# Samirez/Visual_odometry

Hardware: AMD Instinct MI355X
Metric: frame-pairs/sec (1280x720, 2000 ORB feats) (higher is better)
Workload: dtype u8+f32+f64; 1 GPU; seeded synthetic 1280x720 drone flight (256 distinct rendered views, closed loop), 2000 ORB features/frame, 8 levels = BASELINE config 2; chunk of 257 consecutive frames -> 256 pairs (k, k+1) per GPU per step, each frame detected once; detector=orb, distinct_rendered_frames=256, pair_stride=1, contexts_per_gpu=3, keypoint_order=cv2, poly_solver=fast, matcher=crosscheck, matcher_kernel=mfma_fp4, ransac=5-point, conf 0.99, 1 px, seed 2^64-1, <=1000 iters, parallelism=single GPU, pairs_ok_last_step=256

## Files before the change

### visual_odometry_amd/csrc/match_kernels.hip

```cpp
#include "vo_internal.h"
#include <float.h>
#include <limits.h>

#define NN_TILE 256

struct Desc { uint4 a, b; };

__device__ __forceinline__ int hamming(const Desc& x, const uint4& ya, const uint4& yb)
{
    return __popc(x.a.x ^ ya.x) + __popc(x.a.y ^ ya.y) + __popc(x.a.z ^ ya.z) + __popc(x.a.w ^ ya.w) +
           __popc(x.b.x ^ yb.x) + __popc(x.b.y ^ yb.y) + __popc(x.b.z ^ yb.z) + __popc(x.b.w ^ yb.w);
}

#define NN_Q 2
#define NN_ROWS_PER_BLOCK (256 * NN_Q)

template <bool KNN2>
__device__ __forceinline__ void nn_body(const uint8_t* A, int na, const uint8_t* B, int nb,
                                        int* idx, int* dist, int* idx2, int* dist2)
{
    __shared__ uint4 s_b[NN_TILE * 2];
    const int tid = threadIdx.x;
    Desc me[NN_Q];
    int row[NN_Q];
// ... 165 lines not shown
            if (j0 + 16 > nb && j0 + li >= nb) cin = c_bad;
            v4i b[4], acc[MM_RB];
#pragma unroll
            for (int s = 0; s < 4; s++) b[s] = *(const v4i*)(sb + g * 4096 + (4 * s + lg) * 256 + li * 16);
#pragma unroll
            for (int rb = 0; rb < MM_RB; rb++) acc[rb] = __builtin_amdgcn_mfma_i32_16x16x64_i8(a[rb][0], b[0], cin, 0, 0, 0);
#pragma unroll
            for (int s = 1; s < 4; s++)
#pragma unroll
                for (int rb = 0; rb < MM_RB; rb++) acc[rb] = __builtin_amdgcn_mfma_i32_16x16x64_i8(a[rb][s], b[s], acc[rb], 0, 0, 0);
#pragma unroll
            for (int rb = 0; rb < MM_RB; rb++)
#pragma unroll
                for (int r = 0; r < 4; r++) {
                    const int key = acc[rb][r];
                    if (KNN2) best2[rb][r] = max(best2[rb][r], min(best[rb][r], key));
                    best[rb][r] = max(best[rb][r], key);
                }
        }
    }
#undef MM_GLDS

    const size_t o = ((size_t)p * 2 + dir) * kp_cap, o2 = (size_t)p * kp_cap;
#pragma unroll
    for (int rb = 0; rb < MM_RB; rb++)
#pragma unroll
        for (int r = 0; r < 4; r++) {
            int k0 = best[rb][r], k1 = best2[rb][r];
#pragma unroll
            for (int d = 1; d < 16; d <<= 1) {
                const int u0 = __shfl_xor(k0, d, 64), u1 = __shfl_xor(k1, d, 64);
                if (KNN2) k1 = max(max(k1, u1), min(k0, u0));
                k0 = max(k0, u0);
            }
            const int row = wrow0 + rb * 16 + lg * 4 + r;
            if (li == 0 && row < na) {
                pb.nn_idx[o + row] = k0 >= 0 ? MM_S - 1 - k0 % MM_S : -1;
                pb.nn_dist[o + row] = k0 >= 0 ? (512 - k0 / MM_S) >> 1 : INT_MAX;
                if (KNN2) {
                    pb.nn_idx2[o2 + row] = k1 >= 0 ? MM_S - 1 - k1 % MM_S : -1;
                    pb.nn_dist2[o2 + row] = k1 >= 0 ? (512 - k1 / MM_S) >> 1 : INT_MAX;
                }
            }
        }
}

typedef int v8i __attribute__((ext_vector_type(8)));
typedef float v4f __attribute__((ext_vector_type(4)));
#define MF_S 8192
#ifndef MF_STAGE_ROWS
#define MF_STAGE_ROWS 128
#endif
#define MF_LD (MF_STAGE_ROWS * 128 / 16 / MM_THREADS)
template <bool KNN2>
__global__ __launch_bounds__(MM_THREADS) void k_nn_fp4(const uint8_t* desc_x, const int* kp_count, int kp_cap, int cap_x,
                                                PairBuf pb, int dir_first, int row_blocks)
{
    __shared__ __attribute__((aligned(16))) uint8_t s_b[2][MF_STAGE_ROWS * 128];
    const int bid = xcd_tile(blockIdx.x, gridDim.x);
    const int p = bid / row_blocks, dir = dir_first + blockIdx.z;
    const int fa = pb.slots[2 * p + dir], fb = pb.slots[2 * p + (dir ^ 1)];
    const int na = min(kp_count[fa], kp_cap), nb = min(kp_count[fb], kp_cap);
    const int row0 = (bid % row_blocks) * MM_BLOCK_ROWS;
    if (row0 >= na) return;
    const int tid = threadIdx.x, lane = tid & 63, wave = __builtin_amdgcn_readfirstlane(tid >> 6);
    const int li = lane & 15, lg = lane >> 4;
    const uint8_t* A = desc_x + (size_t)fa * cap_x * 256;
    const uint8_t* B = desc_x + (size_t)fb * cap_x * 256;
    const int wrow0 = row0 + wave * MM_WAVE_ROWS;

    v8i a[MM_RB][2];
#pragma unroll
    for (int rb = 0; rb < MM_RB; rb++)
#pragma unroll
        for (int s = 0; s < 2; s++) {
            const v4i v = wrow0 < na ? *(const v4i*)(A + ((size_t)((wrow0 >> 4) + rb) * 8 + 4 * s + lg) * 256 + li * 16) : (v4i){0, 0, 0, 0};
            a[rb][s] = __builtin_shufflevector(v, v, 0, 1, 2, 3, -1, -1, -1, -1);
        }
    const float c_bad = -1.0e9f;
    const float c_lane = (float)(MF_S * 256 + (MF_S - 1) - li);
    v4i best[MM_RB], best2[MM_RB];
#pragma unroll
    for (int rb = 0; rb < MM_RB; rb++) { best[rb] = (v4i){INT_MIN, INT_MIN, INT_MIN, INT_MIN}; best2[rb] = best[rb]; }

    const int nstages = (nb + MF_STAGE_ROWS - 1) / MF_STAGE_ROWS;
    const bool active = wrow0 < na;
    v4f cin = {c_lane, c_lane, c_lane, c_lane};
#define MF_GLDS(stage, buf)                                                                                        \
    _Pragma("unroll") for (int q = 0; q < MF_LD; q++)                                                              \
        __builtin_amdgcn_global_load_lds((const __attribute__((address_space(1))) void*)(B + (size_t)(stage) * (MF_STAGE_ROWS * 128) + (size_t)(q * MM_THREADS + tid) * 16), \
                                         (__attribute__((address_space(3))) void*)(s_b[buf] + (q * MM_THREADS + wave * 64) * 16), 16, 0, 0)
    if (nstages > 0) { MF_GLDS(0, 0); }
    for (int sg = 0; sg < nstages; sg++) {
        asm volatile("s_waitcnt vmcnt(0)" ::: "memory");
        __syncthreads();
        if (sg + 1 < nstages) { MF_GLDS(sg + 1, (sg + 1) & 1); }
        const uint8_t* sb = s_b[sg & 1];
        const int first = sg * (MF_STAGE_ROWS / 16);
        const int ngf = active ? min(MF_STAGE_ROWS / 16, max((nb >> 4) - first, 0)) : 0;
        const bool tail = active && (nb & 15) && first + ngf == (nb >> 4) && ngf < MF_STAGE_ROWS / 16;
        auto group = [&](int g, const v4f& c, v4f (&acc)[MM_RB]) {
            v8i b[2];
#pragma unroll
            for (int s = 0; s < 2; s++) {
                const v4i v = *(const v4i*)(sb + g * 2048 + (4 * s + lg) * 256 + li * 16);
                b[s] = __builtin_shufflevector(v, v, 0, 1, 2, 3, -1, -1, -1, -1);
            }
#pragma unroll
            for (int rb = 0; rb < MM_RB; rb++) acc[rb] = __builtin_amdgcn_mfma_scale_f32_16x16x128_f8f6f4(a[rb][0], b[0], c, 4, 4, 0, 140, 0, 127);
#pragma unroll
            for (int rb = 0; rb < MM_RB; rb++) acc[rb] = __builtin_amdgcn_mfma_scale_f32_16x16x128_f8f6f4(a[rb][1], b[1], acc[rb], 4, 4, 0, 140, 0, 127);
        };
        const v4f sixteen = {16.f, 16.f, 16.f, 16.f};
        int g = 0;
        for (; g + 1 < ngf; g += 2) {
            v4f acc0[MM_RB], acc1[MM_RB];
            const v4f c1 = cin - sixteen;
            group(g, cin, acc0); group(g + 1, c1, acc1);
            cin = c1 - sixteen;
#pragma unroll
            for (int rb = 0; rb < MM_RB; rb++)
#pragma unroll
                for (int r = 0; r < 4; r++) {
                    const int k0 = __float_as_int(acc0[rb][r]), k1 = __float_as_int(acc1[rb][r]);
                    if (KNN2) {
                        best2[rb][r] = max(best2[rb][r], min(best[rb][r], k0));
                        best[rb][r] = max(best[rb][r], k0);
                        best2[rb][r] = max(best2[rb][r], min(best[rb][r], k1));
                        best[rb][r] = max(best[rb][r], k1);
                    } else best[rb][r] = max(max(best[rb][r], k0), k1);
                }
        }
        for (; g < ngf + (tail ? 1 : 0); g++) {
            v4f acc[MM_RB];
            v4f c = cin;
            if (g == ngf) { const float cm = (first + g) * 16 + li >= nb ? c_bad : cin[0]; c = (v4f){cm, cm, cm, cm}; }
            group(g, c, acc);
            cin = cin - sixteen;
#pragma unroll
            for (int rb = 0; rb < MM_RB; rb++)
#pragma unroll
                for (int r = 0; r < 4; r++) {
                    const int key = __float_as_int(acc[rb][r]);
                    if (KNN2) best2[rb][r] = max(best2[rb][r], min(best[rb][r], key));
                    best[rb][r] = max(best[rb][r], key);
                }
        }
    }
#undef MF_GLDS

    const size_t o = ((size_t)p * 2 + dir) * kp_cap, o2 = (size_t)p * kp_cap;
#pragma unroll
    for (int rb = 0; rb < MM_RB; rb++)
#pragma unroll
        for (int r = 0; r < 4; r++) {
            int k0 = best[rb][r], k1 = best2[rb][r];
#pragma unroll
            for (int d = 1; d < 16; d <<= 1) {
                const int u0 = __shfl_xor(k0, d, 64), u1 = __shfl_xor(k1, d, 64);
                if (KNN2) k1 = max(max(k1, u1), min(k0, u0));
                k0 = max(k0, u0);
            }
            const int row = wrow0 + rb * 16 + lg * 4 + r;
            if (li == 0 && row < na) {
                const int i0 = k0 >= 0 ? (int)__int_as_float(k0) : -1, i1 = k1 >= 0 ? (int)__int_as_float(k1) : -1;
                pb.nn_idx[o + row] = i0 >= 0 ? MF_S - 1 - (i0 & (MF_S - 1)) : -1;
                pb.nn_dist[o + row] = i0 >= 0 ? (512 - (i0 >> 13)) >> 1 : INT_MAX;
                if (KNN2) {
                    pb.nn_idx2[o2 + row] = i1 >= 0 ? MF_S - 1 - (i1 & (MF_S - 1)) : -1;
                    pb.nn_dist2[o2 + row] = i1 >= 0 ? (512 - (i1 >> 13)) >> 1 : INT_MAX;
                }
            }
        }
}

void launch_match_nn(hipStream_t s, const uint8_t* desc_x, const int* kp_count, int kp_cap, int cap_x, PairBuf pb, int P,
                     int dirs_mask, int knn2, int fp4)
{
    if (P <= 0) return;
    dim3 block(MM_THREADS);
    const int gx = (kp_cap + MM_BLOCK_ROWS - 1) / MM_BLOCK_ROWS;
    if (fp4) {
        if (knn2) hipLaunchKernelGGL(k_nn_fp4<true>, dim3(gx * P, 1, 1), block, 0, s, desc_x, kp_count, kp_cap, cap_x, pb, 0, gx);
        else if (dirs_mask == 3) hipLaunchKernelGGL(k_nn_fp4<false>, dim3(gx * P, 1, 2), block, 0, s, desc_x, kp_count, kp_cap, cap_x, pb, 0, gx);
        else hipLaunchKernelGGL(k_nn_fp4<false>, dim3(gx * P, 1, 1), block, 0, s, desc_x, kp_count, kp_cap, cap_x, pb, dirs_mask == 2 ? 1 : 0, gx);
        return;
    }
    if (knn2) {
        hipLaunchKernelGGL(k_nn_mfma<true>, dim3(gx * P, 1, 1), block, 0, s, desc_x, kp_count, kp_cap, cap_x, pb, 0, gx);
        return;
    }
    if (dirs_mask == 3) hipLaunchKernelGGL(k_nn_mfma<false>, dim3(gx * P, 1, 2), block, 0, s, desc_x, kp_count, kp_cap, cap_x, pb, 0, gx);
    else if (dirs_mask == 1) hipLaunchKernelGGL(k_nn_mfma<false>, dim3(gx * P, 1, 1), block, 0, s, desc_x, kp_count, kp_cap, cap_x, pb, 0, gx);
    else if (dirs_mask == 2) hipLaunchKernelGGL(k_nn_mfma<false>, dim3(gx * P, 1, 1), block, 0, s, desc_x, kp_count, kp_cap, cap_x, pb, 1, gx);
}

#define L8_STAGE_ROWS 128
#define L8_LD (L8_STAGE_ROWS * 128 / 16 / MM_THREADS)
template <bool KNN2, bool PACKED>
__device__ __forceinline__ void nn_l2i8_body(uint8_t (*s_b)[L8_STAGE_ROWS * 128], const uint8_t* desc_x, const int* norms, int kp_cap, int cap_x,
                                             const PairBuf& pb, int p, int dir, int fa, int fb, int na, int nb, int row0)
{
    constexpr bool packed = PACKED;
    const int tid = threadIdx.x, lane = tid & 63, wave = __builtin_amdgcn_readfirstlane(tid >> 6);
    const int li = lane & 15, lg = lane >> 4;
    const uint8_t* A = desc_x + (size_t)fa * cap_x * 128;
    const uint8_t* B = desc_x + (size_t)fb * cap_x * 128;
    const int* nB = norms + (size_t)fb * cap_x;
    const int wrow0 = row0 + wave * MM_WAVE_ROWS;

    v4i a[MM_RB][2];
#pragma unroll
    for (int rb = 0; rb < MM_RB; rb++)
#pragma unroll
        for (int s = 0; s < 2; s++)
            a[rb][s] = wrow0 < na ? *(const v4i*)(A + ((size_t)((wrow0 >> 4) + rb) * 8 + 4 * s + lg) * 256 + li * 16) : (v4i){0, 0, 0, 0};
    v4i bv[MM_RB], bg[MM_RB], bv2[MM_RB], bg2[MM_RB];
#pragma unroll
    for (int rb = 0; rb < MM_RB; rb++) { bv[rb] = (v4i){INT_MIN, INT_MIN, INT_MIN, INT_MIN}; bg[rb] = (v4i){-1, -1, -1, -1}; bv2[rb] = bv[rb]; bg2[rb] = bg[rb]; }

    const int nstages = (nb + L8_STAGE_ROWS - 1) / L8_STAGE_ROWS;
    const bool active = wrow0 < na;

#define L8_GLDS(stage, buf)                                                                                        \
    _Pragma("unroll") for (int q = 0; q < L8_LD; q++)                                                              \
        __builtin_amdgcn_global_load_lds((const __attribute__((address_space(1))) void*)(B + (size_t)(stage) * (L8_STAGE_ROWS * 128) + (size_t)(q * MM_THREADS + tid) * 16), \
                                         (__attribute__((address_space(3))) void*)(s_b[buf] + (q * MM_THREADS + wave * 64) * 16), 16, 0, 0)
    constexpr int NGS = L8_STAGE_ROWS / 16;
    int nbn[NGS], nbs[NGS];
#define L8_NORMS(stage)                                                                                            \
    _Pragma("unroll") for (int g = 0; g < NGS; g++) {                                                              \
        const int jn = ((stage) * NGS + g) * 16 + li;                                                              \
        nbn[g] = jn < nb ? nB[jn] : 0x3fffffff;                            \
    }
    if (nstages > 0) { L8_NORMS(0); L8_GLDS(0, 0); }
    for (int sg = 0; sg < nstages; sg++) {
        asm volatile("s_waitcnt vmcnt(0)" ::: "memory");
        __syncthreads();
#pragma unroll
        for (int g = 0; g < NGS; g++) nbs[g] = nbn[g];
        if (sg + 1 < nstages) { L8_NORMS(sg + 1); L8_GLDS(sg + 1, (sg + 1) & 1); }
        const uint8_t* sb = s_b[sg & 1];
        const int ng = active ? min(L8_STAGE_ROWS / 16, (nb - sg * L8_STAGE_ROWS + 15) >> 4) : 0;
#pragma unroll
        for (int g = 0; g < NGS; g++) {
            if (g >= ng) break;
            const int gi = sg * (L8_STAGE_ROWS / 16) + g, j = gi * 16 + li;
// ... 74 lines not shown
                pb.nn_dist[o + row] = k0 ? na2 - v0 : INT_MAX;
                if (KNN2) {
                    const int v1 = (int)((unsigned)(k1 >> 32) ^ 0x80000000u), j1 = 0x7fffffff - (int)(k1 & 0xffffffffu);
                    pb.nn_idx2[o2 + row] = k1 ? j1 : -1;
                    pb.nn_dist2[o2 + row] = k1 ? na2 - v1 : INT_MAX;
                }
            }
        }
}

template <bool KNN2>
__global__ __launch_bounds__(MM_THREADS) void k_nn_l2i8(const uint8_t* desc_x, const int* norms, const int* kp_count, int kp_cap, int cap_x,
                                                 PairBuf pb, int dir_first, int row_blocks)
{
    __shared__ __attribute__((aligned(16))) uint8_t s_b[2][L8_STAGE_ROWS * 128];
    const int bid = xcd_tile(blockIdx.x, gridDim.x);
    const int p = bid / row_blocks, dir = dir_first + blockIdx.z;
    const int fa = pb.slots[2 * p + dir], fb = pb.slots[2 * p + (dir ^ 1)];
    const int na = min(kp_count[fa], kp_cap), nb = min(kp_count[fb], kp_cap);
    const int row0 = (bid % row_blocks) * MM_BLOCK_ROWS;
    if (row0 >= na) return;
    if (!KNN2 && nb <= 4096) nn_l2i8_body<false, true>(s_b, desc_x, norms, kp_cap, cap_x, pb, p, dir, fa, fb, na, nb, row0);
    else nn_l2i8_body<KNN2, false>(s_b, desc_x, norms, kp_cap, cap_x, pb, p, dir, fa, fb, na, nb, row0);
}

void launch_match_nn_l2i8(hipStream_t s, const uint8_t* desc_x, const int* norms, const int* kp_count, int kp_cap, int cap_x, PairBuf pb, int P,
                          int dirs_mask, int knn2)
{
    if (P <= 0) return;
    dim3 block(MM_THREADS);
    const int gx = (kp_cap + MM_BLOCK_ROWS - 1) / MM_BLOCK_ROWS;
    if (knn2) hipLaunchKernelGGL(k_nn_l2i8<true>, dim3(gx * P, 1, 1), block, 0, s, desc_x, norms, kp_count, kp_cap, cap_x, pb, 0, gx);
    else if (dirs_mask == 3) hipLaunchKernelGGL(k_nn_l2i8<false>, dim3(gx * P, 1, 2), block, 0, s, desc_x, norms, kp_count, kp_cap, cap_x, pb, 0, gx);
    else hipLaunchKernelGGL(k_nn_l2i8<false>, dim3(gx * P, 1, 1), block, 0, s, desc_x, norms, kp_count, kp_cap, cap_x, pb, dirs_mask == 2 ? 1 : 0, gx);
}

__device__ __forceinline__ int excl_scan_256(int v, int* s_w, int* total)
{
    const int tid = threadIdx.x, lane = tid & 63, wid = tid >> 6;
    int inc = v;
#pragma unroll
    for (int d = 1; d < 64; d <<= 1) { int t = __shfl_up(inc, d, 64); if (lane >= d) inc += t; }
    __syncthreads();
    if (lane == 63) s_w[wid] = inc;
    __syncthreads();
    int off = 0, tot = 0;
#pragma unroll
    for (int w = 0; w < 4; w++) { int x = s_w[w]; if (w < wid) off += x; tot += x; }
    *total = tot;
    return off + inc - v;
}

__global__ __launch_bounds__(256) void k_match_select(const float* kp_xy, const int* kp_count, int kp_cap, PairBuf pb,
                                                      int mode, double ratio, const double* Kd, int l2)
{
    extern __shared__ unsigned long long s_best[];
    __shared__ int s_w[4];
    const int p = blockIdx.x, tid = threadIdx.x;
    const int f1 = pb.slots[2 * p], f2 = pb.slots[2 * p + 1];
    const int nq = min(kp_count[f1], kp_cap), nt = min(kp_count[f2], kp_cap);
    const size_t o0 = ((size_t)p * 2) * kp_cap, o1 = o0 + kp_cap, op = (size_t)p * kp_cap;
    const int* fidx = pb.nn_idx + o0; const int* fdist = pb.nn_dist + o0;
    const int* ridx = pb.nn_idx + o1; const int* rdist = pb.nn_dist + o1;
    if (mode == 1) {
        for (int q = tid; q < nq; q += 256) s_best[q] = ~0ULL;
        __syncthreads();
        for (int t = tid; t < nt; t += 256) {
            const int q = ridx[t];
            if (q >= 0) atomicMin(&s_best[q], ((unsigned long long)(unsigned)rdist[t] << 32) | (unsigned)t);
        }
        __syncthreads();
    }
    const double ifx = 1. / Kd[0], ify = 1. / Kd[4];
    const double bx = -Kd[2] * ifx, by = -Kd[5] * ify;
    const float* xy1 = kp_xy + (size_t)f1 * kp_cap * 2;
    const float* xy2 = kp_xy + (size_t)f2 * kp_cap * 2;
    int out_base = 0;
    for (int base = 0; base < nq; base += 256) {
        const int q = base + tid;
        int t = -1, d = 0;
        if (q < nq && nt > 0) {
            if (mode == 0) { t = fidx[q]; d = fdist[q]; }
            else if (mode == 1) { unsigned long long b = s_best[q]; if (b != ~0ULL) { t = (int)(b & 0xffffffffu); d = (int)(b >> 32); } }
            else if (mode == 2) { t = fidx[q]; d = fdist[q]; if (t >= 0 && ridx[t] != q) t = -1; }
            else {
                const int d1 = pb.nn_dist2[op + q];
                t = fidx[q]; d = fdist[q];
                const float fd = l2 ? sqrtf((float)d) : (float)d, fd1 = l2 ? sqrtf((float)d1) : (float)d1;
                if (nt < 2 || !((double)fd < ratio * (double)fd1)) t = -1;
            }
        }
        int tot;
        const int pos = out_base + excl_scan_256(t >= 0 ? 1 : 0, s_w, &tot);
        if (t >= 0) {
            pb.m_q[op + pos] = q; pb.m_t[op + pos] = t; pb.m_d[op + pos] = l2 ? sqrtf((float)d) : (float)d;
            const double u1 = (double)xy1[2 * q], v1 = (double)xy1[2 * q + 1];
            const double u2 = (double)xy2[2 * t], v2 = (double)xy2[2 * t + 1];
            const size_t o = (op + pos) * 2;
            pb.px1[o] = u1; pb.px1[o + 1] = v1; pb.px2[o] = u2; pb.px2[o + 1] = v2;
            pb.xn1[o] = u1 * ifx + bx; pb.xn1[o + 1] = v1 * ify + by;
            pb.xn2[o] = u2 * ifx + bx; pb.xn2[o + 1] = v2 * ify + by;
        }
        out_base += tot;
    }
    if (tid == 0) {
        pb.m_count[p] = out_base;
        pb.res[p].n_kp1 = nq; pb.res[p].n_kp2 = nt; pb.res[p].n_match = out_base;
    }
}

void launch_match_select(hipStream_t s, const float* kp_xy, const int* kp_count, int kp_cap, PairBuf pb, int P,
                         int mode, double ratio, const double* K, int l2)
{
    if (P <= 0) return;
    size_t shmem = mode == 1 ? (size_t)kp_cap * 8 : 8;
    if (shmem > 64 * 1024) (void)hipFuncSetAttribute((const void*)k_match_select, hipFuncAttributeMaxDynamicSharedMemorySize, (int)shmem);
    hipLaunchKernelGGL(k_match_select, dim3(P), dim3(256), shmem, s, kp_xy, kp_count, kp_cap, pb, mode, ratio, K, l2);
}

#define L2_TILE 32
template <int DIM, bool KNN2>
__global__ __launch_bounds__(64) void k_nn_l2(const float* A, int na, const float* B, int nb, int dim, unsigned long long* key, int split_rows)
{
    extern __shared__ float s_t[];
    const int row = blockIdx.x * 64 + threadIdx.x;
    const bool live = row < na;
    const float* a = A + (size_t)(live ? row : 0) * dim;
    float areg[DIM > 0 ? DIM : 1];
    if (DIM > 0) {
#pragma unroll
        for (int k = 0; k < DIM; k++) areg[k] = a[k];
    }
    float best = FLT_MAX, best2 = FLT_MAX;
    int bi = -1, bi2 = -1;
    const int b_lo = blockIdx.y * split_rows, b_hi = min(nb, b_lo + split_rows);
    for (int base = b_lo; base < b_hi; base += L2_TILE) {
        const int rows = min(L2_TILE, b_hi - base);
        __syncthreads();
        for (int i = threadIdx.x; i < rows * dim; i += 64) s_t[i] = B[(size_t)base * dim + i];
        __syncthreads();
        for (int r = 0; r < rows; r++) {
            const float* b = s_t + r * dim;
            float acc[4][4];
#pragma unroll
            for (int m = 0; m < 4; m++)
#pragma unroll
                for (int l = 0; l < 4; l++) acc[m][l] = 0.f;
            int j = 0;
            if (DIM > 0) {
#pragma unroll
                for (int jj = 0; jj <= DIM - 16; jj += 16)
#pragma unroll
                    for (int m = 0; m < 4; m++)
#pragma unroll
                        for (int l = 0; l < 4; l++) { const float t = areg[jj + 4 * m + l] - b[jj + 4 * m + l]; const float p = t * t; acc[m][l] = p + acc[m][l]; }
                j = DIM - DIM % 16;
            } else {
                for (; j <= dim - 16; j += 16)
#pragma unroll
                    for (int m = 0; m < 4; m++)
#pragma unroll
                        for (int l = 0; l < 4; l++) { const float t = a[j + 4 * m + l] - b[j + 4 * m + l]; const float p = t * t; acc[m][l] = p + acc[m][l]; }
            }
            float s[4];
#pragma unroll
            for (int l = 0; l < 4; l++) s[l] = ((acc[0][l] + acc[1][l]) + acc[2][l]) + acc[3][l];
            float d = (s[0] + s[2]) + (s[1] + s[3]);
            for (; j < dim; j++) { const float t = (DIM > 0 ? areg[DIM > 0 ? min(j, DIM - 1) : 0] : a[j]) - b[j]; const float p = t * t; d = d + p; }
            d = sqrtf(d);
            if (KNN2) {
// ... 88 lines not shown
```

### visual_odometry_amd/csrc/vo_api.hip

```cpp
#include "vo_internal.h"
#include <float.h>
#include <math.h>
#include <stdio.h>
#include <stdlib.h>
#include <string.h>
#include <vector>
#include <algorithm>

#define MAX_EVENTS 160

struct DevList {
    struct Entry { void* p; bool pinned; };
    std::vector<Entry> ptrs;
    DevList() = default;
    DevList(const DevList&) = delete;
    DevList& operator=(DevList&& o) noexcept { if (this != &o) { release(); ptrs.swap(o.ptrs); } return *this; }
    ~DevList() { release(); }
    template <typename T> hipError_t alloc(T** p, size_t n) { return keep(hipMalloc((void**)p, (n ? n : 1) * sizeof(T)), (void**)p, false); }
    template <typename T> hipError_t alloc_pinned(T** p, size_t n)
    {
        return keep(hipHostMalloc((void**)p, (n ? n : 1) * sizeof(T), hipHostMallocDefault), (void**)p, true);
    }
    void release()
    {
// ... 222 lines not shown
        lv.sel_chunk_base = sc;
        sc += trows;
        lv.cand_off = co;
        lv.cand_cap = align_up(want + (want > 1024 ? want : 1024), 8);
        co += lv.cand_cap;
    }
    g->frame_bytes = align_up(off, 256);
    g->ftiles_total = ft; g->btiles_total = bt; g->dtiles_total = dt;
    g->cand_total = co;
    g->sel_chunks_total = sc;
    g->kp_cap = align_up(p->nfeatures + (p->nfeatures / 8 > 256 ? p->nfeatures / 8 : 256), 8);
    return VO_OK;
}

static void build_lin_tab(int ssize, int dsize, int* ofs, uint16_t* c1, int* pmin, int* pmax)
{
    const double inv_scale = (double)dsize / (double)ssize;
    const double scale = 1.0 / inv_scale;
    int minofst = 0, maxofst = dsize;
    for (int val = 0; val < dsize; val++) {
        volatile double fval = scale * ((double)val + 0.5);
        fval = fval - 0.5;
        const double fv = fval;
        const int ival = cv_floor_d(fv);
        ofs[val] = 0; c1[val] = 0;
        if (ival >= 0 && ssize > 1) {
            if (ival < ssize - 1) {
                ofs[val] = ival;
                volatile double fr = fv - (double)ival;
                fr = fr * 256.0;
                c1[val] = (uint16_t)lrint((double)fr);
            } else {
                ofs[val] = ssize - 1;
                if (val < maxofst) maxofst = val;
            }
        } else if (val + 1 > minofst) minofst = val + 1;
    }
    *pmin = minofst; *pmax = maxofst;
}

static hipError_t alloc_pairbuf(DevList& mem, PairBuf& pb, int P, int cap, bool with_pose_mask)
{
    hipError_t e;
    const size_t pc = (size_t)P * cap;
    pb = PairBuf{};
#define A_(field, n) if ((e = mem.alloc(&pb.field, (n))) != hipSuccess) return e
    A_(slots, (size_t)P * 2); A_(nn_idx, pc * 2); A_(nn_dist, pc * 2); A_(nn_idx2, pc); A_(nn_dist2, pc);
    A_(m_q, pc); A_(m_t, pc); A_(m_d, pc); A_(m_count, (size_t)P);
    A_(px1, pc * 2); A_(px2, pc * 2); A_(xn1, pc * 2); A_(xn2, pc * 2);
    A_(mask, pc); A_(models, (size_t)P * 64 * 90);
    A_(in1, pc * 2); A_(in2, pc * 2); A_(ipx1, pc * 2); A_(ipx2, pc * 2);
    A_(res, (size_t)P); A_(X, pc * 4);
    if (with_pose_mask) { A_(pose_mask, pc); }
#undef A_
    return hipSuccess;
}

static int alloc_cv2(vo_ctx* ctx)
{
    if (ctx->cv2_ready) return VO_OK;
    const PyrGeom& g = ctx->g;
    Cv2Buf& cb = ctx->cv2;
    int off = 0;
    for (int l = 0; l < g.nlevels; l++) {
        const int px8 = g.lv[l].w * g.lv[l].h / 8 + 1024;
        cb.all_off[l] = off;
        cb.all_cap[l] = align_up(px8 > g.lv[l].cand_cap ? px8 : g.lv[l].cand_cap, 8);
        off += cb.all_cap[l];
    }
    cb.all_total = off;
    const size_t F = (size_t)ctx->max_frames, n = F * off;
    DevList& m = ctx->orb_mem;
    HIPCHK(m.alloc(&cb.all_pos, n)); HIPCHK(m.alloc(&cb.all_resp, n)); HIPCHK(m.alloc(&cb.work, n));
    HIPCHK(m.alloc(&cb.lpos, n)); HIPCHK(m.alloc(&cb.rpos, n));
    HIPCHK(m.alloc(&cb.all_count, F * VO_MAX_LEVELS)); HIPCHK(m.alloc(&cb.ones, F * VO_MAX_LEVELS));
    HIPCHK(m.alloc(&cb.chunk_count, F * (size_t)(g.sel_chunks_total + 1)));
    std::vector<int> ones(F * VO_MAX_LEVELS, 1);
    HIPCHK(hipMemcpy(cb.ones, ones.data(), ones.size() * sizeof(int), hipMemcpyHostToDevice));
    HIPCHK(hipMemset(cb.all_count, 0, F * VO_MAX_LEVELS * sizeof(int)));
    HIPCHK(hipDeviceSynchronize());
    ctx->cv2_ready = true;
    return VO_OK;
}

static void free_config(vo_ctx* c)
{
    c->configured = c->cv2_ready = false;
    c->orb_mem.release();
    c->pb_mem.release();
    c->pb_pairs = c->pb_cap = 0;
    clear_last_run(c);
}

static void comm_release(vo_ctx* ctx);
static int sift_frames_upload_enqueue(vo_ctx* ctx, const uint8_t* frames, int F, int row_stride, int64_t frame_stride, int first_slot);
static int sift_frames_detect_enqueue(vo_ctx* ctx, int first_slot, int F);

extern "C" int vo_version(void) { return 120; }

extern "C" int vo_create(int device_id, vo_ctx** out)
{
    if (!out) return VO_ERR_INVALID;
    *out = nullptr;
    int ndev = 0;
    if (hipGetDeviceCount(&ndev) != hipSuccess || device_id < 0 || device_id >= ndev) return VO_ERR_HIP;
    vo_ctx* ctx = new vo_ctx();
// ... 478 lines not shown
        if (lw < 1 || lh < 1) return VO_ERR_INVALID;
        total += (int64_t)lw * lh;
    }
    return total;
}

extern "C" int vo_stage_pyramid(vo_ctx* ctx, const uint8_t* img, int h, int w, int channels, int row_stride,
                                const vo_orb_params* params, uint8_t* out_packed)
{
    int rc = stage_common(ctx, img, h, w, channels, row_stride, params, 0);
    return rc ? rc : download_packed(ctx, ctx->pyr, out_packed);
}

extern "C" int vo_stage_fast_scores(vo_ctx* ctx, const uint8_t* img, int h, int w, int channels, int row_stride,
                                    const vo_orb_params* params, uint8_t* out_packed)
{
    int rc = stage_common(ctx, img, h, w, channels, row_stride, params, 1);
    return rc ? rc : download_packed(ctx, ctx->score, out_packed);
}

extern "C" int vo_stage_blur(vo_ctx* ctx, const uint8_t* img, int h, int w, int channels, int row_stride,
                             const vo_orb_params* params, uint8_t* out_packed)
{
    int rc = stage_common(ctx, img, h, w, channels, row_stride, params, 2);
    return rc ? rc : download_packed(ctx, ctx->blur, out_packed);
}

#define RNG_TAB_N 8192
static int ensure_rng(vo_ctx* ctx, uint64_t seed)
{
    if (ctx->rng_valid && ctx->rng_seed == seed) return VO_OK;
    if (!ctx->rng_tab) HIPCHK(ctx->mem.alloc(&ctx->rng_tab, RNG_TAB_N));
    if (!ctx->rng_host) HIPCHK(ctx->mem.alloc_pinned(&ctx->rng_host, RNG_TAB_N));
    HIPCHK(hipStreamSynchronize(ctx->stream));
    uint32_t* tab = ctx->rng_host;
    uint64_t st = seed ? seed : 0xffffffffULL;
    for (int i = 0; i < RNG_TAB_N; i++) {
        st = (uint64_t)(uint32_t)st * 4164903690ULL + (uint32_t)(st >> 32);
        tab[i] = (uint32_t)st;
    }
    HIPCHK(hipMemcpyAsync(ctx->rng_tab, tab, RNG_TAB_N * sizeof(uint32_t), hipMemcpyHostToDevice, ctx->stream));
    ctx->rng_seed = seed; ctx->rng_valid = true;
    return VO_OK;
}

static int map_select_mode(int match_mode) { return match_mode == 0 ? 2 : match_mode == 2 ? 1 : 3; }

static int run_pairs(vo_ctx* ctx, PairBuf pb, const uint8_t* desc, const uint8_t* desc_x, const float* kp_xy, const int* kp_count, int cap,
                     int P, int select_mode, double ratio, const RansacParams& rp, bool do_geometry, bool want_points, int descx_fp4,
                     const int* l2_norms = nullptr)
{
    hipStream_t s = ctx->stream;
    HIPCHK(hipMemsetAsync(pb.res, 0, (size_t)P * sizeof(vo_pair_result), s));
    if (l2_norms) {
        StageTimer t(ctx, ST_MATCH_NN);
        const int cx = desc_x_rows(cap);
        const int dirs = select_mode == 0 ? 1 : select_mode == 1 ? 2 : 3;
        if (select_mode == 3) launch_match_nn_l2i8(s, desc_x, l2_norms, kp_count, cap, cx, pb, P, 1, 1);
        else launch_match_nn_l2i8(s, desc_x, l2_norms, kp_count, cap, cx, pb, P, dirs, 0);
    } else {
        StageTimer t(ctx, ST_MATCH_NN);
        const int cx = desc_x_rows(cap);
        const int dirs = select_mode == 0 ? 1 : select_mode == 1 ? 2 : 3;
        if (ctx->matcher_kernel == 1 || cap >= 16129) {
            if (select_mode == 3) launch_match_nn_popcount(s, desc, kp_count, cap, pb, P, 1, 1);
            else launch_match_nn_popcount(s, desc, kp_count, cap, pb, P, dirs, 0);
        } else if (select_mode == 3) launch_match_nn(s, desc_x, kp_count, cap, cx, pb, P, 1, 1, descx_fp4);
        else launch_match_nn(s, desc_x, kp_count, cap, cx, pb, P, dirs, 0, descx_fp4);
    }
    { StageTimer t(ctx, ST_MATCH_SELECT); launch_match_select(s, kp_xy, kp_count, cap, pb, P, select_mode, ratio, ctx->dK, l2_norms ? 1 : 0); }
    if (!do_geometry) return VO_OK;
    { int rc = ensure_rng(ctx, rp.seed); if (rc) return rc; }
    { StageTimer t(ctx, ST_RANSAC); launch_ransac(s, pb, cap, P, rp, ctx->rng_tab, RNG_TAB_N); }
    { StageTimer t(ctx, ST_POSE); launch_pose(s, pb, cap, P, rp); }
    if (want_points) { StageTimer t(ctx, ST_TRIANGULATE); launch_triangulate_pairs(s, pb, cap, P, rp); }
    return VO_OK;
}

static int pairs_enqueue(vo_ctx* ctx, const int32_t* pair_slots, int B, const double* K, const vo_pair_opts* opts,
                         vo_pair_result* results, double* X, int32_t x_cap, bool* whole_x_out)
{
    const Batch b = batch(ctx);
    if (!b.ready) FAIL(VO_ERR_NOT_CONFIGURED, "vo_batch_configure has not been called");
    if (!pair_slots || !K || !opts || !results || B < 0 || B > b.max_pairs) FAIL(VO_ERR_INVALID, "bad pair batch arguments");
    if (opts->match_mode < 0 || opts->match_mode > 2) FAIL(VO_ERR_INVALID, "match_mode must be 0, 1 or 2");
    if (!(opts->ransac_prob > 0 && opts->ransac_prob < 1)) FAIL(VO_ERR_INVALID, "ransac_prob must be in (0, 1)");
    for (int i = 0; i < 2 * B; i++)
        if (pair_slots[i] < 0 || pair_slots[i] >= b.max_frames) FAIL(VO_ERR_INVALID, "pair slot %d out of range", pair_slots[i]);
    *whole_x_out = false;
    clear_last_run(ctx);
    const bool wp = opts->want_points != 0;
    auto done = [&]() {
        ctx->last.pairs = B;
        ctx->last.slots.assign(pair_slots, pair_slots + 2 * (size_t)B);
        ctx->last.points = wp;
        return VO_OK;
    };
    if (B == 0) return done();
    HIPCHK(hipSetDevice(ctx->device));
    hipStream_t s = ctx->stream;
    const int cap = b.kp_cap;
    HIPCHK(hipMemcpyAsync(ctx->pb.slots, pair_slots, (size_t)B * 2 * sizeof(int), hipMemcpyHostToDevice, s));
    HIPCHK(hipMemcpyAsync(ctx->dK, K, 9 * sizeof(double), hipMemcpyHostToDevice, s));
    RansacParams rp{};
    rp.prob = opts->ransac_prob; rp.thresh_px = opts->ransac_thresh; rp.max_iters = opts->ransac_max_iters;
    rp.seed = opts->ransac_seed; rp.dist_thresh = opts->pose_dist_thresh; rp.dk_early = ctx->dk_early;
    memcpy(rp.K, K, sizeof(rp.K));
    int rc = run_pairs(ctx, ctx->pb, b.desc, b.desc_x, b.kp_xy, b.kp_count, cap, B, map_select_mode(opts->match_mode), opts->ratio, rp, true, wp,
                       b.fp4, b.norms);
    if (rc) return rc;
    HIPCHK(hipGetLastError());
    HIPCHK(hipMemcpyAsync(results, ctx->pb.res, (size_t)B * sizeof(vo_pair_result), hipMemcpyDeviceToHost, s));
    const bool whole_x = X && wp && x_cap == cap;
    if (X && wp && x_cap < 1) FAIL(VO_ERR_INVALID, "x_cap must be positive");
    if (whole_x) HIPCHK(hipMemcpyAsync(X, ctx->pb.X, (size_t)B * 4 * cap * sizeof(double), hipMemcpyDeviceToHost, s));
    *whole_x_out = whole_x;
    return done();
}

extern "C" int vo_pairs_run(vo_ctx* ctx, const int32_t* pair_slots, int B, const double* K, const vo_pair_opts* opts,
                            vo_pair_result* results, double* X, int32_t x_cap)
{
    if (!ctx) return VO_ERR_INVALID;
// ... 1486 lines not shown
```

### visual_odometry_amd/csrc/vo_internal.h

```cpp
#pragma once
#include <hip/hip_runtime.h>
#include <stdint.h>
#include "../../include/vo_hip.h"

enum {
    ST_GRAY = 0, ST_RESIZE, ST_FAST, ST_SELECT_FAST, ST_HARRIS, ST_SELECT_HARRIS, ST_ANGLE,
    ST_BLUR, ST_BRIEF, ST_MATCH_NN, ST_MATCH_SELECT, ST_RANSAC, ST_POSE, ST_TRIANGULATE,
    ST_MISC, ST_RESERVED, ST_SIFT_SCALE, ST_SIFT_EXTREMA, ST_SIFT_ORIENT, ST_SIFT_SORT, ST_SIFT_DESC, ST_CV2_ORDER, ST_GATHER, ST_RESERVED2
};

struct LevelGeom {
    int w, h, stride, off;
    int quota;
    float scale;
    int ftile_base, ftiles_x;
    int fox, foy;
    int dtile_base, dtiles_x;
    int btile_base, btiles_x;
    int cand_off, cand_cap;
    int sel_chunk_base;
};

struct PyrGeom {
    int nlevels, frame_bytes;
// ... 17 lines not shown
    const int* yofs; const uint16_t* yc1;
    int min_x, max_x, min_y, max_y;
    int direct;
};

#ifndef FAST_TW
#define FAST_TW 112
#endif
#ifndef FAST_TH
#define FAST_TH 20
#endif
#define BLUR_TW 128
#ifndef BLUR_TH
#define BLUR_TH 48
#endif
#define FAST_LISTCAP ((FAST_TW / 2) * (FAST_TH / 2))

struct FrameFeat {
    uint32_t* cand_pos;
    float*    cand_resp;
    int*      cand_count;
    uint32_t* kp_pos;
    int*      kp_level;
    float*    kp_resp;
    float*    kp_angle;
    float*    kp_xy;
    float*    kp_size;
    uint8_t*  desc;
    int*      kp_count;
    int*      flags;
    uint32_t* hist;
    uint32_t* tile_list;
    int*      tile_count;
};

struct Cv2Buf {
    uint32_t* all_pos;
    float*    all_resp;
    int*      all_count;
    int*      chunk_count;
    int*      ones;
    uint2*    work;
    uint32_t* lpos;
    uint32_t* rpos;
    int all_off[VO_MAX_LEVELS], all_cap[VO_MAX_LEVELS], all_total;
};

struct PairBuf {
    int*      slots;
    int*      nn_idx;
    int*      nn_dist;
    int*      nn_idx2;
    int*      nn_dist2;
    int*      m_q;
    int*      m_t;
    float*    m_d;
    int*      m_count;
    double*   px1;
    double*   px2;
    double*   xn1;
    double*   xn2;
    uint8_t*  mask;
    double*   models;
    double*   in1;
    double*   in2;
    double*   ipx1;
    double*   ipx2;
    vo_pair_result* res;
    double*   X;
    uint8_t*  pose_mask;
};

struct RansacParams {
    double prob, thresh_px;
    int max_iters;
    uint64_t seed;
    double K[9];
    double dist_thresh;
    int dk_early;
};

const char* rccl_load(void);
const char* rccl_unique_id(uint8_t* id128);
const char* rccl_comm_init(void** comm, const uint8_t* id128, int rank, int world);
void rccl_comm_destroy(void* comm);
const char* rccl_comm_count(void* comm, int* n);
const char* rccl_all_gather_f64(void* comm, const double* send, double* recv, size_t count, hipStream_t s);
void launch_pack_records(hipStream_t s, const vo_pair_result* res, int B, int valid, double* rec);

void launch_gray(hipStream_t s, const uint8_t* src, int channels, int row_stride, int64_t frame_stride,
                 uint8_t* pyr, const PyrGeom& g, int F);
void launch_gray_plain(hipStream_t s, const uint8_t* src, int channels, int row_stride, int64_t frame_stride,
                       uint8_t* dst, int w, int h, int dstride, int64_t dframe, int F);
void launch_resize(hipStream_t s, uint8_t* pyr, const PyrGeom& g, int level, const ResizeTab& tab, int F);
void launch_fast(hipStream_t s, const uint8_t* pyr, uint8_t* score, uint32_t* hist, const PyrGeom& g, int F,
                 uint32_t* tile_list, int* tile_count);
void launch_select_fast(hipStream_t s, const PyrGeom& g, FrameFeat ff, int F, int* thr, int* chunk_count,
                        const uint32_t* tile_list, const int* tile_count);
void launch_harris(hipStream_t s, const uint8_t* pyr, const PyrGeom& g, FrameFeat ff, int F);
void launch_all_winners(hipStream_t s, const PyrGeom& g, FrameFeat ff, const Cv2Buf& cb, int F, const uint32_t* tile_list, const int* tile_count);
void launch_cv2_order(hipStream_t s, const PyrGeom& g, FrameFeat ff, Cv2Buf cb, int F, const int* kept);
void launch_retain_raw(hipStream_t s, const float* resp, int n, int n_points, uint2* a, uint32_t* lpos, uint32_t* rpos,
                       int* order, int* n_out);
void launch_select_harris(hipStream_t s, const PyrGeom& g, FrameFeat ff, int F, float* thr, int* kept);
void launch_angle(hipStream_t s, const uint8_t* pyr, const PyrGeom& g, FrameFeat ff, int F);
void launch_resize_linear(hipStream_t st, const uint8_t* src, int sw, int sh, int cn, int sstride, int64_t sframe,
// ... 3 lines not shown
                        int isx, int isy, const int* xsi, const float* xal, const int* xst, const int* ysi, const float* yal, const int* yst);
#define SIFT_IMG_BORDER 5
#define SIFT_MAX_INTERP_STEPS 5
#define SIFT_MAX_OCT 16
#define SIFT_MAX_TAPS 64
struct SiftGeom {
    int nOct, nLayers;
    int w[SIFT_MAX_OCT], h[SIFT_MAX_OCT], stride[SIFT_MAX_OCT];
    size_t plane[SIFT_MAX_OCT];
    size_t goff[SIFT_MAX_OCT];
    size_t gframe;
};
struct SiftCand { int o, layer, r, c; };
struct SiftKp { float x, y, size, angle, response; int octave; };
struct SiftSurv { SiftKp kp; int o, layer, r, c; };
struct SiftExpTab { float tab[64]; };
int launch_sb_sweep_base(hipStream_t s, const uint8_t* img, int channels, int row_stride, int64_t frame_stride, int sw, int sh,
                         float* dstG, size_t g_fs, int stride, int F, const float* taps, int ntaps);
int launch_sb_sweep(hipStream_t s, const float* src, size_t src_fs, float* dstG, size_t g_fs, int w, int h, int stride, int F,
                    const float* taps, int ntaps, float* dstH = nullptr, size_t h_fs = 0, int hstride = 0, int hw = 0, int hh = 0);
void launch_sb_extrema(hipStream_t s, const SiftGeom& P, const float* gauss, int o, float threshold, SiftCand* cand, int* counts, int cap, int F);
void launch_sb_refine_orient(hipStream_t s, const SiftGeom& P, const float* gauss, const SiftCand* cand, int cand_cap, float contrastThr,
                             float edgeThr, float sigma, const SiftExpTab& E, SiftSurv* surv, int surv_cap, SiftKp* kps, int kp_cap, int* counts, int F, int waves);
void launch_sb_sort_emit(hipStream_t s, const SiftKp* kps, int kp_cap, int* counts, int* rank , void* rank_tmp , SiftKp* sorted,
                         SiftKp* out, int out_cap, int* out_count, int* out_flags, int cand_cap, int surv_cap, int F);
void launch_sb_descriptor(hipStream_t s, const SiftGeom& P, const float* gauss, const SiftKp* kps, int kp_cap, const int* counts, const SiftExpTab& E,
                          uint8_t* desc, uint8_t* desc_x, int cap_x, int* norms, int* flags, int first_slot, int F, int waves);
void launch_sb_unpack(hipStream_t s, const SiftKp* kps, int kp_cap, const int* counts, int first_slot, float* kp_xy, float* kp_size, float* kp_angle,
                      float* kp_resp, int* kp_oct, int* kp_count, const int* fin_count, const int* fin_flags, int* flags, int F);
void launch_match_nn_l2i8(hipStream_t s, const uint8_t* desc_x, const int* norms, const int* kp_count, int kp_cap, int cap_x, PairBuf pb, int P,
                          int dirs_mask, int knn2);

#include "jpeg_host.h"
void launch_jpeg_decode(hipStream_t s, const uint8_t* blob, JpegImage* imgs, const JpegTables* tabs, int F, uint8_t* clean, uint32_t* rst,
                        int16_t* coef, uint8_t* planes, uint8_t* out, int max_blocks, int max_w, int max_h, bool gray = false,
                        bool packed_tables = false ,
                        hipEvent_t coef_cleared = nullptr );

void launch_pnp_ransac(hipStream_t s, const double* obj, const double* img, const int* offsets, int B, const double* Kd,
                       int iterations, double reproj_err, double confidence, uint64_t seed, const uint32_t* rng_tab, int rng_n,
                       int refine_cv2, double* rvec, double* tvec, uint8_t* mask, int* ninl, int* status);
void launch_rodrigues(hipStream_t s, const double* in, int in_is_matrix, double* out);
void launch_blur(hipStream_t s, const uint8_t* pyr, uint8_t* blur, const PyrGeom& g, int F);
void launch_brief(hipStream_t s, const uint8_t* blur, const PyrGeom& g, FrameFeat ff, int F, uint8_t* desc_x, int cap_x, int fp4);

__device__ __forceinline__ int xcd_tile(int b, int n)
{
    const int q = n >> 3, r = n & 7, x = b & 7, k = b >> 3;
    return (x < r ? x * (q + 1) : r * (q + 1) + (x - r) * q) + k;
}

static inline int desc_x_rows(int kp_cap) { return (kp_cap + 255) & ~255; }
void launch_desc_expand(hipStream_t s, const uint8_t* desc, const int* kp_count, int kp_cap, int cap_x, uint8_t* desc_x, int F, int fp4);
void launch_match_nn(hipStream_t s, const uint8_t* desc_x, const int* kp_count, int kp_cap, int cap_x, PairBuf pb, int P,
                     int dirs_mask, int knn2, int fp4);
void launch_match_nn_popcount(hipStream_t s, const uint8_t* desc, const int* kp_count, int kp_cap, PairBuf pb, int P,
                              int dirs_mask, int knn2);
void launch_match_select(hipStream_t s, const float* kp_xy, const int* kp_count, int kp_cap, PairBuf pb, int P,
                         int mode, double ratio, const double* K, int l2 = 0);

size_t nn_l2_knn2_keys(int na, int nb);
void launch_nn_l2_knn2(hipStream_t s, const float* A, int na, const float* B, int nb, int dim, int* idx, float* dist, unsigned long long* part);
void launch_nn_l2(hipStream_t s, const float* A, int na, const float* B, int nb, int dim, int* idx, float* dist, unsigned long long* key);

void launch_ransac(hipStream_t s, PairBuf pb, int kp_cap, int P, RansacParams rp, const uint32_t* rng_tab, int rng_n);
void launch_pose(hipStream_t s, PairBuf pb, int kp_cap, int P, RansacParams rp);
void launch_triangulate_pairs(hipStream_t s, PairBuf pb, int kp_cap, int P, RansacParams rp);
void launch_triangulate_raw(hipStream_t s, const double* P1, const double* P2, const double* x1, const double* x2,
                            int M, double* X);
void launch_five_point_raw(hipStream_t s, const double* x1, const double* x2, double* E, int* nm, int dk_early);
void launch_reprojection(hipStream_t s, const double* poses, int ncam, const double* points, int npt, const int* obs_cam,
                         const int* obs_pt, const double* obs_xy, int nobs, const double* Kd, double threshold,
                         double* sqerr, uint8_t* keep, int* bad);
struct ChainBuf {
    unsigned long long* parent;
    uint8_t* in_map;
    double*  map_pt;
    double*  cam;
    int*     cam_ok;
    double*  obj;
    double*  img;
    int*     off;
    double*  rvec; double* tvec;
    uint8_t* pmask;
    int*     pninl; int* pstatus;
    double*  P1; double* P2;
    double*  Xw;
    int*     alive;
    int*     n_corr; int* n_inl; int* status; int* n_map;
    double*  poses;
    int*     map_count;
};
void launch_chain_link(hipStream_t s, PairBuf pb, int kp_cap, int P, ChainBuf cb);
void launch_chain_init(hipStream_t s, PairBuf pb, int kp_cap, ChainBuf cb);
void launch_chain_gather(hipStream_t s, PairBuf pb, int kp_cap, int p, int F, ChainBuf cb);
void launch_chain_pose(hipStream_t s, PairBuf pb, int p, const double* Kd, ChainBuf cb);
void launch_chain_triangulate(hipStream_t s, PairBuf pb, int kp_cap, int p, ChainBuf cb);
void launch_chain_insert(hipStream_t s, PairBuf pb, int kp_cap, int p, int F, double max_norm, ChainBuf cb);
void launch_tracks(hipStream_t s, const int* pair_frames, const int* match_off, const int* mq, const int* mt, int P, int max_m,
                   int F, int cap, unsigned long long* parent, int* root_frame, int* root_idx, int* hops, int* bad);
```

Baseline: 88340 frame-pairs/s.

## Derive reverse-direction NN from forward fp4 matmul via column maxima

```diff
diff --git a/visual_odometry_amd/csrc/match_kernels.hip b/visual_odometry_amd/csrc/match_kernels.hip
--- a/visual_odometry_amd/csrc/match_kernels.hip
+++ b/visual_odometry_amd/csrc/match_kernels.hip
@@ -241,17 +241,11 @@
 #define MF_STAGE_ROWS 128
 #endif
 #define MF_LD (MF_STAGE_ROWS * 128 / 16 / MM_THREADS)
-template <bool KNN2>
-__global__ __launch_bounds__(MM_THREADS) void k_nn_fp4(const uint8_t* desc_x, const int* kp_count, int kp_cap, int cap_x,
-                                                PairBuf pb, int dir_first, int row_blocks)
-{
-    __shared__ __attribute__((aligned(16))) uint8_t s_b[2][MF_STAGE_ROWS * 128];
-    const int bid = xcd_tile(blockIdx.x, gridDim.x);
-    const int p = bid / row_blocks, dir = dir_first + blockIdx.z;
-    const int fa = pb.slots[2 * p + dir], fb = pb.slots[2 * p + (dir ^ 1)];
-    const int na = min(kp_count[fa], kp_cap), nb = min(kp_count[fb], kp_cap);
-    const int row0 = (bid % row_blocks) * MM_BLOCK_ROWS;
-    if (row0 >= na) return;
+typedef float v2f __attribute__((ext_vector_type(2)));
+template <bool KNN2, bool COLS>
+__device__ __forceinline__ void nn_fp4_body(uint8_t (*s_b)[MF_STAGE_ROWS * 128], int* s_col, const uint8_t* desc_x, int kp_cap, int cap_x,
+                                            const PairBuf& pb, int p, int dir, int fa, int fb, int na, int nb, int rbk, int row0)
+{
     const int tid = threadIdx.x, lane = tid & 63, wave = __builtin_amdgcn_readfirstlane(tid >> 6);
     const int li = lane & 15, lg = lane >> 4;
     const uint8_t* A = desc_x + (size_t)fa * cap_x * 256;
@@ -271,6 +265,41 @@
     v4i best[MM_RB], best2[MM_RB];
 #pragma unroll
     for (int rb = 0; rb < MM_RB; rb++) { best[rb] = (v4i){INT_MIN, INT_MIN, INT_MIN, INT_MIN}; best2[rb] = best[rb]; }
+
+    v2f coff[MM_RB][2];
+    if (COLS) {
+#pragma unroll
+        for (int rb = 0; rb < MM_RB; rb++)
+#pragma unroll
+            for (int h = 0; h < 2; h++)
+#pragma unroll
+                for (int e = 0; e < 2; e++) {
+                    const int i = wrow0 + rb * 16 + lg * 4 + 2 * h + e;
+                    coff[rb][h][e] = i < na ? (float)(MF_S - 1 - i) : -16777216.f;
+                }
+        for (int c = tid; c < ((nb + 15) & ~15); c += MM_THREADS) s_col[c] = INT_MIN;
+    }
+    auto colmax = [&](const v4f (&acc)[MM_RB]) -> int {
+        int x[16];
+#pragma unroll
+        for (int rb = 0; rb < MM_RB; rb++)
+#pragma unroll
+            for (int h = 0; h < 2; h++) {
+                const v2f t = (v2f){acc[rb][2 * h], acc[rb][2 * h + 1]} + coff[rb][h];
+                x[rb * 4 + 2 * h] = __float_as_int(t.x); x[rb * 4 + 2 * h + 1] = __float_as_int(t.y);
+            }
+        const int m0 = max(max(x[0], x[1]), x[2]), m1 = max(max(x[3], x[4]), x[5]), m2 = max(max(x[6], x[7]), x[8]);
+        const int m3 = max(max(x[9], x[10]), x[11]), m4 = max(max(x[12], x[13]), x[14]);
+        return max(max(max(m0, m1), m2), max(max(m3, m4), x[15]));
+    };
+    auto colflush = [&](int c0, int c1, int j0, bool two) {
+        const auto h = __builtin_amdgcn_permlane32_swap(c0, c1, false, false);
+        const int m = max((int)h[0], (int)h[1]);
+        const auto q = __builtin_amdgcn_permlane16_swap(m, m, false, false);
+        const int v = max((int)q[0], (int)q[1]);
+        if (!(lane & 16) && (two || lane < 32))
+            asm volatile("ds_max_i32 %0, %1" :: "v"((unsigned)(uintptr_t)(__attribute__((address_space(3))) int*)(s_col + j0 + (lane >> 5) * 16 + li)), "v"(v) : "memory");
+    };
 
     const int nstages = (nb + MF_STAGE_ROWS - 1) / MF_STAGE_ROWS;
     const bool active = wrow0 < na;
@@ -319,6 +348,7 @@
                         best[rb][r] = max(best[rb][r], k1);
                     } else best[rb][r] = max(max(best[rb][r], k0), k1);
                 }
+            if (COLS) colflush(colmax(acc0), colmax(acc1), (first + g) * 16, true);
         }
         for (; g < ngf + (tail ? 1 : 0); g++) {
             v4f acc[MM_RB];
@@ -334,6 +364,7 @@
                     if (KNN2) best2[rb][r] = max(best2[rb][r], min(best[rb][r], key));
                     best[rb][r] = max(best[rb][r], key);
                 }
+            if (COLS) colflush(colmax(acc), INT_MIN, (first + g) * 16, false);
         }
     }
 #undef MF_GLDS
@@ -361,27 +392,64 @@
                 }
             }
         }
-}
-
-void launch_match_nn(hipStream_t s, const uint8_t* desc_x, const int* kp_count, int kp_cap, int cap_x, PairBuf pb, int P,
-                     int dirs_mask, int knn2, int fp4)
-{
-    if (P <= 0) return;
+    if (COLS) {
+        asm volatile("s_waitcnt lgkmcnt(0)" ::: "memory");
+        __syncthreads();
+        int* part = pb.nn_colkey + ((size_t)p * rbk + row0 / MM_BLOCK_ROWS) * kp_cap;
+        for (int c = tid; c < nb; c += MM_THREADS) {
+            const int k = s_col[c];
+            part[c] = k >= 0 ? (int)__int_as_float(k) - (MF_S - 1 - c) : -1;
+        }
+    }
+}
+
+template <bool KNN2>
+__global__ __launch_bounds__(MM_THREADS) void k_nn_fp4(const uint8_t* desc_x, const int* kp_count, int kp_cap, int cap_x,
+                                                PairBuf pb, int dir_first, int row_blocks, int cols)
+{
+    __shared__ __attribute__((aligned(16))) uint8_t s_b[2][MF_STAGE_ROWS * 128];
+    extern __shared__ int s_col[];
+    const int bid = xcd_tile(blockIdx.x, gridDim.x);
+    const int p = bid / row_blocks, dir = dir_first + blockIdx.z;
+    const int fa = pb.slots[2 * p + dir], fb = pb.slots[2 * p + (dir ^ 1)];
+    const int na = min(kp_count[fa], kp_cap), nb = min(kp_count[fb], kp_cap);
+    const int row0 = (bid % row_blocks) * MM_BLOCK_ROWS;
+    if (row0 >= na) return;
+    if (!KNN2 && cols) nn_fp4_body<false, true>(s_b, s_col, desc_x, kp_cap, cap_x, pb, p, dir, fa, fb, na, nb, row_blocks, row0);
+    else nn_fp4_body<KNN2, false>(s_b, s_col, desc_x, kp_cap, cap_x, pb, p, dir, fa, fb, na, nb, row_blocks, row0);
+}
+
+#define NN_COLS_MAX 4096
+size_t nn_colkey_ints(int P, int kp_cap)
+{
+    return kp_cap <= NN_COLS_MAX ? (size_t)P * ((kp_cap + MM_BLOCK_ROWS - 1) / MM_BLOCK_ROWS) * kp_cap : 0;
+}
+
+int launch_match_nn(hipStream_t s, const uint8_t* desc_x, const int* kp_count, int kp_cap, int cap_x, PairBuf pb, int P,
+                    int dirs_mask, int knn2, int fp4)
+{
+    if (P <= 0) return 0;
     dim3 block(MM_THREADS);
     const int gx = (kp_cap + MM_BLOCK_ROWS - 1) / MM_BLOCK_ROWS;
     if (fp4) {
-        if (knn2) hipLaunchKernelGGL(k_nn_fp4<true>, dim3(gx * P, 1, 1), block, 0, s, desc_x, kp_count, kp_cap, cap_x, pb, 0, gx);
-        else if (dirs_mask == 3) hipLaunchKernelGGL(k_nn_fp4<false>, dim3(gx * P, 1, 2), block, 0, s, desc_x, kp_count, kp_cap, cap_x, pb, 0, gx);
-        else hipLaunchKernelGGL(k_nn_fp4<false>, dim3(gx * P, 1, 1), block, 0, s, desc_x, kp_count, kp_cap, cap_x, pb, dirs_mask == 2 ? 1 : 0, gx);
-        return;
+        if (knn2) hipLaunchKernelGGL(k_nn_fp4<true>, dim3(gx * P, 1, 1), block, 0, s, desc_x, kp_count, kp_cap, cap_x, pb, 0, gx, 0);
+        else if (dirs_mask == 3 && pb.nn_colkey && kp_cap <= NN_COLS_MAX) {
+            const size_t shmem = (size_t)((kp_cap + 15) & ~15) * sizeof(int);
+            hipLaunchKernelGGL(k_nn_fp4<false>, dim3(gx * P, 1, 1), block, shmem, s, desc_x, kp_count, kp_cap, cap_x, pb, 0, gx, 1);
+            return 1;
+        }
+        else if (dirs_mask == 3) hipLaunchKernelGGL(k_nn_fp4<false>, dim3(gx * P, 1, 2), block, 0, s, desc_x, kp_count, kp_cap, cap_x, pb, 0, gx, 0);
+        else hipLaunchKernelGGL(k_nn_fp4<false>, dim3(gx * P, 1, 1), block, 0, s, desc_x, kp_count, kp_cap, cap_x, pb, dirs_mask == 2 ? 1 : 0, gx, 0);
+        return 0;
     }
     if (knn2) {
         hipLaunchKernelGGL(k_nn_mfma<true>, dim3(gx * P, 1, 1), block, 0, s, desc_x, kp_count, kp_cap, cap_x, pb, 0, gx);
-        return;
+        return 0;
     }
     if (dirs_mask == 3) hipLaunchKernelGGL(k_nn_mfma<false>, dim3(gx * P, 1, 2), block, 0, s, desc_x, kp_count, kp_cap, cap_x, pb, 0, gx);
     else if (dirs_mask == 1) hipLaunchKernelGGL(k_nn_mfma<false>, dim3(gx * P, 1, 1), block, 0, s, desc_x, kp_count, kp_cap, cap_x, pb, 0, gx);
     else if (dirs_mask == 2) hipLaunchKernelGGL(k_nn_mfma<false>, dim3(gx * P, 1, 1), block, 0, s, desc_x, kp_count, kp_cap, cap_x, pb, 1, gx);
+    return 0;
 }
 
 #define L8_STAGE_ROWS 128
@@ -562,7 +630,7 @@
 }
 
 __global__ __launch_bounds__(256) void k_match_select(const float* kp_xy, const int* kp_count, int kp_cap, PairBuf pb,
-                                                      int mode, double ratio, const double* Kd, int l2)
+                                                      int mode, double ratio, const double* Kd, int l2, int col_parts)
 {
     extern __shared__ unsigned long long s_best[];
     __shared__ int s_w[4];
@@ -572,6 +640,26 @@
     const size_t o0 = ((size_t)p * 2) * kp_cap, o1 = o0 + kp_cap, op = (size_t)p * kp_cap;
     const int* fidx = pb.nn_idx + o0; const int* fdist = pb.nn_dist + o0;
     const int* ridx = pb.nn_idx + o1; const int* rdist = pb.nn_dist + o1;
+    if (col_parts) {
+        const int* part = pb.nn_colkey + (size_t)p * ((kp_cap + MM_BLOCK_ROWS - 1) / MM_BLOCK_ROWS) * kp_cap;
+        const int rbk = (nq + MM_BLOCK_ROWS - 1) / MM_BLOCK_ROWS;
+        for (int t0 = tid; t0 < nt; t0 += 4 * 256) {
+            int k[4] = {-1, -1, -1, -1};
+#pragma unroll 4
+            for (int g = 0; g < rbk; g++)
+#pragma unroll
+                for (int u = 0; u < 4; u++) k[u] = max(k[u], part[(size_t)g * kp_cap + min(t0 + u * 256, nt - 1)]);
+#pragma unroll
+            for (int u = 0; u < 4; u++) {
+                const int t = t0 + u * 256;
+                if (t < nt) {
+                    pb.nn_idx[o1 + t] = k[u] >= 0 ? MF_S - 1 - (k[u] & (MF_S - 1)) : -1;
+                    pb.nn_dist[o1 + t] = k[u] >= 0 ? (512 - (k[u] >> 13)) >> 1 : INT_MAX;
+                }
+            }
+        }
+        __syncthreads();
+    }
     if (mode == 1) {
         for (int q = tid; q < nq; q += 256) s_best[q] = ~0ULL;
         __syncthreads();
@@ -620,12 +708,12 @@
 }
 
 void launch_match_select(hipStream_t s, const float* kp_xy, const int* kp_count, int kp_cap, PairBuf pb, int P,
-                         int mode, double ratio, const double* K, int l2)
+                         int mode, double ratio, const double* K, int l2, int col_parts)
 {
     if (P <= 0) return;
     size_t shmem = mode == 1 ? (size_t)kp_cap * 8 : 8;
     if (shmem > 64 * 1024) (void)hipFuncSetAttribute((const void*)k_match_select, hipFuncAttributeMaxDynamicSharedMemorySize, (int)shmem);
-    hipLaunchKernelGGL(k_match_select, dim3(P), dim3(256), shmem, s, kp_xy, kp_count, kp_cap, pb, mode, ratio, K, l2);
+    hipLaunchKernelGGL(k_match_select, dim3(P), dim3(256), shmem, s, kp_xy, kp_count, kp_cap, pb, mode, ratio, K, l2, col_parts);
 }
 
 #define L2_TILE 32
diff --git a/visual_odometry_amd/csrc/vo_api.hip b/visual_odometry_amd/csrc/vo_api.hip
--- a/visual_odometry_amd/csrc/vo_api.hip
+++ b/visual_odometry_amd/csrc/vo_api.hip
@@ -298,6 +298,7 @@
     A_(in1, pc * 2); A_(in2, pc * 2); A_(ipx1, pc * 2); A_(ipx2, pc * 2);
     A_(res, (size_t)P); A_(X, pc * 4);
     if (with_pose_mask) { A_(pose_mask, pc); }
+    if (const size_t n = nn_colkey_ints(P, cap)) { A_(nn_colkey, n); }
 #undef A_
     return hipSuccess;
 }
@@ -882,6 +883,7 @@
 {
     hipStream_t s = ctx->stream;
     HIPCHK(hipMemsetAsync(pb.res, 0, (size_t)P * sizeof(vo_pair_result), s));
+    int col_parts = 0;
     if (l2_norms) {
         StageTimer t(ctx, ST_MATCH_NN);
         const int cx = desc_x_rows(cap);
@@ -896,9 +898,9 @@
             if (select_mode == 3) launch_match_nn_popcount(s, desc, kp_count, cap, pb, P, 1, 1);
             else launch_match_nn_popcount(s, desc, kp_count, cap, pb, P, dirs, 0);
         } else if (select_mode == 3) launch_match_nn(s, desc_x, kp_count, cap, cx, pb, P, 1, 1, descx_fp4);
-        else launch_match_nn(s, desc_x, kp_count, cap, cx, pb, P, dirs, 0, descx_fp4);
-    }
-    { StageTimer t(ctx, ST_MATCH_SELECT); launch_match_select(s, kp_xy, kp_count, cap, pb, P, select_mode, ratio, ctx->dK, l2_norms ? 1 : 0); }
+        else col_parts = launch_match_nn(s, desc_x, kp_count, cap, cx, pb, P, dirs, 0, descx_fp4);
+    }
+    { StageTimer t(ctx, ST_MATCH_SELECT); launch_match_select(s, kp_xy, kp_count, cap, pb, P, select_mode, ratio, ctx->dK, l2_norms ? 1 : 0, col_parts); }
     if (!do_geometry) return VO_OK;
     { int rc = ensure_rng(ctx, rp.seed); if (rc) return rc; }
     { StageTimer t(ctx, ST_RANSAC); launch_ransac(s, pb, cap, P, rp, ctx->rng_tab, RNG_TAB_N); }
diff --git a/visual_odometry_amd/csrc/vo_internal.h b/visual_odometry_amd/csrc/vo_internal.h
--- a/visual_odometry_amd/csrc/vo_internal.h
+++ b/visual_odometry_amd/csrc/vo_internal.h
@@ -93,6 +93,7 @@
     int*      nn_dist;
     int*      nn_idx2;
     int*      nn_dist2;
+    int*      nn_colkey;
     int*      m_q;
     int*      m_t;
     float*    m_d;
@@ -202,12 +203,14 @@
 
 static inline int desc_x_rows(int kp_cap) { return (kp_cap + 255) & ~255; }
 void launch_desc_expand(hipStream_t s, const uint8_t* desc, const int* kp_count, int kp_cap, int cap_x, uint8_t* desc_x, int F, int fp4);
-void launch_match_nn(hipStream_t s, const uint8_t* desc_x, const int* kp_count, int kp_cap, int cap_x, PairBuf pb, int P,
-                     int dirs_mask, int knn2, int fp4);
+int launch_match_nn(hipStream_t s, const uint8_t* desc_x, const int* kp_count, int kp_cap, int cap_x, PairBuf pb, int P,
+                    int dirs_mask, int knn2, int fp4);
+size_t nn_colkey_ints(int P, int kp_cap);
 void launch_match_nn_popcount(hipStream_t s, const uint8_t* desc, const int* kp_count, int kp_cap, PairBuf pb, int P,
                               int dirs_mask, int knn2);
 void launch_match_select(hipStream_t s, const float* kp_xy, const int* kp_count, int kp_cap, PairBuf pb, int P,
-                         int mode, double ratio, const double* K, int l2 = 0);
+                         int mode, double ratio, const double* K, int l2 = 0,
+                         int col_parts = 0);
 
 size_t nn_l2_knn2_keys(int na, int nb);
 void launch_nn_l2_knn2(hipStream_t s, const float* A, int na, const float* B, int nb, int dim, int* idx, float* dist, unsigned long long* part);
```

Result: faster. 90580 frame-pairs/s (median of 6 runs) (+2.5%).
